# BrandonHanx/TextReID

Measured on AMD Instinct MI355X. Metric: image-text pairs/sec (train), CLIP-RN50 + BiGRU MoCo step, bs128/GPU, higher is better.
Workload: dtype f32; 1 GPU; configs[1]: CLIP-RN50 + GRU, bs128/GPU, 384x128 images, 64-token captions, MoCo queue 8192, fp32, 1xMI355X; random-init weights, synthetic inputs resident in HBM; global_batch=128, parallelism=dp1, optimizer=Adam (fused multi-tensor), step_launch=eager launches, four streams (chosen by the probe over the recorded step)

## Files before the change

include/textreid_hip.h:

```cpp
#ifndef TEXTREID_HIP_H
#define TEXTREID_HIP_H

#include <stdint.h>

#ifdef __cplusplus
extern "C" {
#endif
#if defined(__GNUC__) || defined(__clang__)
#pragma GCC visibility push(default)
#endif

#define TRID_OK 0
#define TRID_E_INVALID (-1)
#define TRID_E_UNSUPPORTED (-2)

#define TRID_VERSION 100

int trid_version(void);
const char* trid_arch(void);
const char* trid_last_error_string(void);

enum {
    TRID_A_KC = 0,
    TRID_A_MC = 1,
// ... 108 lines not shown
int trid_conv3x3_s2_eval_p16_ok(int B, int H, int W, int Cin, int Cout);
int trid_subsample2_p16(const void* x, void* out, int B, int H, int W, int C, void* stream);
int trid_global_avgpool_p16(const void* x, const float* x_amax, float* out, int B, int HW, int C, void* stream);

int trid_stem_conv1_f32(const float* img, const float* w, float* y, float* stats, int B, int Hi, int Wi, void* stream);
int trid_stem_conv1_eval_p16(const float* img, const float* w, const float* bn_scale, const float* bn_shift, void* out,
                             const float* eval_coef, const float* eval_tin, float* out_bound, float* out_tmax, int B, int Hi, int Wi,
                             int relu, void* stream);
int trid_conv3x3_wgrad_halo_rows(int H, int W, int Cin, int Cout);
int trid_conv3x3_wgrad_halo_slabs(void);
int trid_conv3x3_wgrad_halo_p16(const void* dy, const float* dy_amax, const void* x, const float* x_amax, float* dw, float* slabs,
                                int B, int H, int W, int Cin, int Cout, void* stream);
int trid_stem_conv1_wgrad_slabs(void);
int trid_stem_conv1_wgrad_f32(const float* img, const float* dy, float* dw, float* slabs, int B, int Hi, int Wi, void* stream);
int trid_conv3x3_halo_rows(int H, int W, int Cin, int Cout);
int trid_conv3x3_halo_p16(const void* x, const float* x_amax, const void* w, const float* w_amax, float* y, float* stats,
                          int B, int H, int W, int Cin, int Cout, int chunks_per_image, void* stream);
int trid_conv3x3_halo_eval_p16(const void* x, const float* x_amax, const void* w, const float* w_amax, const float* bn_scale,
                               const float* bn_shift, void* out, const float* eval_coef, const float* eval_tin, float* out_bound,
                               float* out_tmax, int B, int H, int W, int Cin, int Cout, int relu, int pool, void* stream);
int trid_conv3x3_halo_eval_pool_ok(int H, int W, int Cin, int Cout);

long long trid_bn_finalize_ws_bytes(void);
int trid_bn_finalize_f32(const float* partials, int nparts, int rows_per_part, long long M, int C,
                         const float* gamma, const float* beta, float* running_mean, float* running_var,
                         float momentum, float eps, float* mean, float* invstd, float* scale, float* shift,
                         void* ws, void* stream);
int trid_bn_eval_coeffs_f32(const float* gamma, const float* beta, const float* running_mean,
                            const float* running_var, float eps, float* scale, float* shift, int C, void* stream);
int trid_bn_eval_bound_f32(const float* partials, int nparts, int C, const float* scale, const float* shift, int relu,
                           float* bound, void* stream);
int trid_eval_bound_coefs_f32(const long long* table, int n_tensors, float* coef, void* stream);
int trid_bn_apply_f32(const float* y, const float* scale, const float* shift, const float* res,
                      const float* rscale, const float* rshift, float* out, long long M, int C, int relu,
                      uint64_t* relu_mask, float* amax, void* stream);
int trid_bn_apply_pool2_f32(const float* y, const float* scale, const float* shift, float* out, int B, int H,
                            int W, int C, int relu, float* amax, void* stream);
int trid_bn_finalize_minmax_f32(const float* partials, int nparts, int rows_per_part, long long M, int C,
                                const float* gamma, const float* beta, float* running_mean, float* running_var,
                                float momentum, float eps, float* mean, float* invstd, float* scale, float* shift,
                                int relu, float* amax_out, void* ws, void* stream);
int trid_bn_apply_p16_f32(const void* y, int y_fmt, const float* scale, const float* shift, const void* res, const float* rscale,
                          const float* rshift, int res_fmt, const float* res_amax, void* out, int fmt, long long M, int C,
                          int relu, uint64_t* relu_mask, const float* bound_a, const float* bound_b, float* bound_sum,
                          void* stream);
int trid_bn_apply_pool2_p16_f32(const void* y, const float* scale, const float* shift, int in_fmt, const float* in_amax,
                                void* out, int fmt, int B, int H, int W, int C, int relu, const float* bound, void* stream);
int trid_avgpool2_bwd_f32(const void* g, void* dx, int B, int H, int W, int C, int accumulate, int fmt, void* stream);

long long trid_bn_bwd_ws_floats(int C);
long long trid_bn_bwd_fused_ws_floats(long long M, int C);
int trid_bn_bwd_final_f32(const float* ws, const float* ws2, long long M, int C, const float* scale, float* dgamma, float* dbeta,
                          float* bound, void* stream);
int trid_bn_bwd_reduce_f32(const float* g, const float* y, const float* act, const float* mean,
                           const float* invstd, const float* scale, const float* shift, int mask_mode,
                           int pooled, int B, int H, int W, int C, float* dgamma, float* dbeta, float* ws,
                           void* stream);
int trid_bn_bwd_apply_f32(const float* g, const float* y, const float* act, const float* mean,
                          const float* invstd, const float* scale, const float* shift, const float* dgamma,
                          const float* dbeta, int mask_mode, int pooled, int B, int H, int W, int C, float* dy,
                          float* dres, float* amax, void* stream);
int trid_bn_bwd_reduce_bound_f32(const float* g, const float* y, const float* act, const float* mean,
                                 const float* invstd, const float* scale, const float* shift, int mask_mode, int pooled,
                                 int B, int H, int W, int C, float* dgamma, float* dbeta, float* ws, float* bound,
                                 void* stream);
int trid_bn_bwd_reduce_g_f32(const void* g, int g_fmt, const void* y, int y_fmt, const float* act, const float* mean,
                             const float* invstd, const float* scale, const float* shift, int mask_mode,
                             int pooled, int B, int H, int W, int C, float* dgamma, float* dbeta, float* ws,
                             void* stream);
int trid_bn_bwd_apply_p16_f32(const void* g, int g_fmt, const void* y, int y_fmt, const float* act, const float* mean, const float* invstd,
                              const float* scale, const float* shift, const float* dgamma, const float* dbeta,
                              int mask_mode, int pooled, int B, int H, int W, int C, void* dy, int fmt, void* dres,
                              const float* bound, void* stream);

int trid_bn_bwd_dual_reduce_bound_f32(const float* g, const uint64_t* relu_bits, const float* y1, const float* y2, const float* mean1,
                                      const float* invstd1, const float* scale1, const float* mean2, const float* invstd2,
                                      const float* scale2, long long M, int C, float* dgamma1, float* dgamma2, float* dbeta,
                                      float* dbeta2, float* ws, float* bound1, float* bound2, void* stream);
int trid_bn_bwd_dual_apply_p16_f32(const float* g, const uint64_t* relu_bits, const float* y1, const float* y2, const float* mean1,
                                   const float* invstd1, const float* scale1, const float* mean2, const float* invstd2,
                                   const float* scale2, const float* dgamma1, const float* dgamma2, const float* dbeta, long long M,
                                   int C, void* dy1, void* dy2, const float* bound1, const float* bound2, void* stream);

int trid_attnpool_tokens_f32(const float* x, const float* pos, float* tok, int B, int T, int C, int ldt,
                             void* stream);
int trid_attnpool_tokens_fmt_f32(const void* x, int x_fmt, const float* x_amax, const float* pos, float* tok, int B, int T,
                                 int C, int ldt, void* stream);
int trid_attnpool_tokens_bwd_f32(const float* dtok, float* dx, float* dpos, int B, int T, int C, int ldt,
                                 void* stream);
int trid_softmax_rows_f32(float* s, long long rows, int n, int ld, void* stream);
int trid_softmax_rows_bwd_f32(const float* p, const float* dp, float* ds, long long rows, int n, int ld,
                              void* stream);
int trid_colsum_f32(const float* x, float* out, long long M, int N, long long ld, int accumulate, void* stream);

int trid_embedding_gather_f32(const float* table, const int64_t* tokens, float* x, int B, int L, int ldtok, int E,
                              long long vocab, void* stream);
int trid_embedding_bwd_f32(const float* dX, const int64_t* tokens, int B, int L, int ldtok, int E, float* dtable,
                           long long vocab, long long padding_idx, void* stream);
int trid_gru_cell_fwd_f32(const float* gi, const float* gh, float* h, const int64_t* lengths, float* gates,
                          float* hprev, float* maxv, int32_t* argt, int s, int Lmax, int L, int B, int Hd,
                          long long gates_dstride, long long hprev_dstride, void* stream);
int trid_gru_max_init_f32(float* maxv, int32_t* argt, const int64_t* lengths, int Lmax, const int64_t* lmax_dev, int B,
                          int Hd, void* stream);
int trid_gru_cell_bwd_f32(const float* dout, const int32_t* argt, const float* gates, const float* hprev,
                          const int64_t* lengths, float* dh, float* dGi, float* dgh, int s, int Lmax, int L,
                          int B, int Hd, long long gates_dstride, long long hprev_dstride, long long dgh_dstride,
                          void* stream);

long long trid_gru_whh_image_bytes(int H);
int trid_gru_step_workgroups(int B, int H);
int trid_gru_pack_whh_f16(const float* w_hh, const float* w_amax, void* img_fwd, void* img_bwd, int H, void* stream);
int trid_gru_step_fwd_f32(const void* img_fwd, const float* w_amax, const void* hp_in, void* hp_out, float* h,
                          const float* gi, const int64_t* lengths, float* gates, float* hprev, float* maxv,
                          int32_t* argt, int s, int Lmax, int L, int B, int Bp, int H, long long gates_dstride,
                          long long hprev_dstride, void* stream);
int trid_gru_step_bwd_f32(const void* img_bwd, const float* w_amax, const float* dgh_in, const float* amax_in,
                          float* amax_out, const float* dout, const int32_t* argt, const float* gates,
                          const float* hprev, const int64_t* lengths, float* dh, float* dGi, float* dgh_out, int s,
                          int Lmax, int L, int B, int H, long long gates_dstride, long long hprev_dstride,
                          long long dgh_dstride, void* stream);

int trid_gru_step_seq_fwd_f32(const void* img_fwd, const float* w_amax, const void* hp_in, void* hp_out, float* h,
                              const float* gi, const int64_t* lengths, float* gates, float* hprev, float* yseq, int s,
                              int Lmax, int L, int B, int Bp, int H, long long gates_dstride, long long hprev_dstride,
                              void* stream);
int trid_gru_step_seq_bwd_f32(const void* img_bwd, const float* w_amax, const float* dgh_in, const float* amax_in,
                              float* amax_out, const float* dyseq, const float* gates, const float* hprev,
                              const int64_t* lengths, float* dh, float* dGi, float* dgh_out, int s, int Lmax, int L, int B,
                              int H, long long gates_dstride, long long hprev_dstride, long long dgh_dstride, void* stream);
int trid_gru_cell_seq_fwd_f32(const float* gi, const float* gh, float* h, const int64_t* lengths, float* gates,
                              float* hprev, float* yseq, int s, int Lmax, int L, int B, int Hd, long long gates_dstride,
                              long long hprev_dstride, void* stream);
int trid_gru_cell_seq_bwd_f32(const float* dyseq, const float* gates, const float* hprev, const int64_t* lengths,
                              float* dh, float* dGi, float* dgh, int s, int Lmax, int L, int B, int Hd,
                              long long gates_dstride, long long hprev_dstride, long long dgh_dstride, void* stream);
int trid_dropout_seq_fwd_f32(const float* y, float* x, uint8_t* keep, long long n, float p, const int64_t* state,
                             long long draw, void* stream);
int trid_dropout_seq_bwd_f32(float* dx, const uint8_t* keep, long long n, float p, void* stream);
int trid_dropout_advance(int64_t* state, long long draws, void* stream);

int trid_l2norm_rows_f32(const float* x, float* y, float* inv_norm, long long rows, int C, float eps, void* stream);
int trid_l2norm_rows_bwd_f32(const float* dy, const float* y, const float* inv_norm, float* dx, long long rows,
                             int C, int accumulate, void* stream);
int trid_queue_hit_mask(const int64_t* id_queue, const int64_t* ids, uint8_t* flag, int K, int B, void* stream);
long long trid_infonce_ws_floats(int B, int K);
int trid_infonce_rows_f32(float* S, const float* pos, const uint8_t* hit, float* loss_rows, float* dpos, int B,
                          int K, int ldS, float invT, float gscale, float* ws, void* stream);
int trid_infonce_queue_rows_f32(float* S, const float* q, const float* key, const uint8_t* hit, float* loss_rows,
                                float* dq0, int B, int K, int ldS, int C, float invT, float gscale, float* ws,
                                void* stream);
long long trid_queue_nce_ws_floats(int B, int K, int C, int nwg_hint);
int trid_queue_nce_f32(const float* v_q, const float* t_q, const float* v_key, const float* t_key,
                       const float* t_queue, const float* v_queue, const int64_t* id_queue, const int64_t* ids,
                       float* loss_rows, float* dq, int B, int K, int C, float invT, float logit_bound, float gscale,
                       int precision, int nwg_hint, float* ws, unsigned int* ticket, float* loss, float loss_scale,
                       void* stream);
int trid_amax_f32(const float* x, long long n, float* out, void* stream);
int trid_amax_multi_f32(const float* const* ptrs, const long long* sizes, int n_tensors, float* out, void* stream);
long long trid_image_pipeline_ws_bytes(int B, int max_src_h, int W);
int trid_image_pipeline_u8(const uint8_t* src, const long long* offset, const int* hw, const int* xbounds,
                           const int* xweights, const int* ybounds, const int* yweights, const int* params, int B,
                           int H, int W, int KX, int KY, int max_src_h, int pad, const float* mean3_std3_erase3_host,
                           uint8_t* ws, float* out, void* stream);
int trid_relu_bwd_f32(const float* dy, const float* act, float* dx, long long n, void* stream);
int trid_rowdot_f32(const float* x, const float* y, float* out, long long rows, int C, void* stream);
int trid_rowscale_add_f32(const float* s, const float* y, float* dx, long long rows, int C, int accumulate,
// ... 89 lines not shown
```

textreid_amd/backbones/m_resnet.py:

```python

import logging
import math
import os
from collections import OrderedDict

import torch
from torch import nn

from .. import ops


class Bottleneck(nn.Module):
    expansion = 4

    def __init__(self, inplanes, planes, stride=1):
        super().__init__()
        self.conv1 = nn.Conv2d(inplanes, planes, 1, bias=False)
        self.bn1 = nn.BatchNorm2d(planes)
        self.conv2 = nn.Conv2d(planes, planes, 3, padding=1, bias=False)
        self.bn2 = nn.BatchNorm2d(planes)
        self.avgpool = nn.AvgPool2d(stride) if stride > 1 else nn.Identity()
        self.conv3 = nn.Conv2d(planes, planes * 4, 1, bias=False)
        self.bn3 = nn.BatchNorm2d(planes * 4)
        self.relu = nn.ReLU(inplace=True)
# ... 372 lines not shown
    G[id(blk.conv3.weight)] = ws.run(lambda d_, x_: ops.conv1x1_wgrad(d_, x_, prec=P, aa=a_dyc, ba=a_ab), dyc, ab, keep=(a_dyc, a_ab)).view_as(blk.conv3.weight)
    a_dyb = ar.slot()
    dyb, dg, db, _ = ops.bn_bwd(dab, yb, stb, None, 1, pooled=stride > 1, amax=a_dyb)
    G[id(blk.bn2.weight)], G[id(blk.bn2.bias)] = dg, db
    planes = blk.conv2.out_channels
    wbt = ops.weight_transpose(_w3x3(blk.conv2), planes, 9, planes, flip=True)
    daa = ops.conv3x3(dyb, wbt, prec=P, aa=a_dyb, ba=ar.wam(blk.conv2))
    G[id(blk.conv2.weight)] = _g3x3(ws.run(lambda d_, x_: ops.conv3x3_wgrad(d_, x_, prec=P, aa=a_dyb, ba=a_aa), dyb, aa, keep=(a_dyb, a_aa)), planes, planes)
    a_dya = ar.slot()
    dya, dg, db, _ = ops.bn_bwd(daa, ya, sta, None, 1, amax=a_dya)
    G[id(blk.bn1.weight)], G[id(blk.bn1.bias)] = dg, db
    wa = blk.conv1.weight.view(blk.conv1.out_channels, -1)
    if has_down:
        wd = blk.downsample[1].weight.view(blk.downsample[1].out_channels, -1)
        dxd = ops.matmul_nn(dyd.view(-1, dyd.shape[-1]), wd, prec=P, aa=a_dyd, ba=ar.wam(blk.downsample[1])).view(xd.shape)
        G[id(blk.downsample[1].weight)] = ws.run(lambda d_, x_: ops.conv1x1_wgrad(d_, x_, prec=P, aa=a_dyd, ba=a_xd), dyd, xd, keep=(a_dyd, a_xd)).view_as(blk.downsample[1].weight)
        dx = ops.avgpool2_bwd(dxd) if stride > 1 else dxd
    else:
        dx = dres
    ops.matmul_nn(dya.view(-1, dya.shape[-1]), wa, out=dx.view(-1, dx.shape[-1]), accumulate=True, prec=P, aa=a_dya, ba=ar.wam(blk.conv1))
    G[id(blk.conv1.weight)] = ws.run(lambda d_, x_: ops.conv1x1_wgrad(d_, x_, prec=P, aa=a_dya, ba=ax), dya, x, keep=(a_dya, ax)).view_as(blk.conv1.weight)
    return dx


def block_forward_p16(blk, x, WP, dev, training, save, nbt, masks=None):
    assert training
    stride = blk.stride
    fmt = x.fmt

    def fin(bn, parts, M, relu):
        if fmt == 2:
            return _bn_coeffs(bn, parts, M, True, nbt), None
        bound = ops.amax_slot(dev)
        return _finalize_minmax(bn, parts, M, relu, bound, nbt), bound

    ya, pa = ops.conv_p16(x, WP[id(blk.conv1.weight)])
    Ma = ya.numel() // ya.shape[-1]
    sta, a_aa = fin(blk.bn1, pa, Ma, True)
    aa = ops.bn_apply_p16(ya, sta, a_aa, relu=True, fmt=fmt)
    yb, pb = ops.conv_p16(aa, WP[id(blk.conv2.weight)], conv3=True)
    stb, a_ab = fin(blk.bn2, pb, Ma, True)
    ab = ops.bn_apply_pool2_p16(yb, stb, a_ab, relu=True, fmt=fmt) if stride > 1 else ops.bn_apply_p16(yb, stb, a_ab, relu=True, fmt=fmt)
    Mc = ab.data.numel() // ab.shape[-1]
    xd = yd = std = None
    if blk.downsample is None and fmt == 1 and not save and ops.conv1x1_bn_res_ok(Mc, blk.conv3.out_channels, ab.shape[-1]):
        pc = ops.conv1x1_stats_p16(ab, WP[id(blk.conv3.weight)])
        stc, a_c = fin(blk.bn3, pc, Mc, False)
        out, rmask, yc = ops.conv1x1_bn_res_p16(ab, WP[id(blk.conv3.weight)], stc, a_c, x, relu=True, want_mask=save, keep_y=save)
        rec = (x, ya, sta, aa, yb, stb, ab, yc, stc, xd, yd, std, rmask) if save else None
        if masks is not None:
            masks.extend([aa.unpack() > 0, ab.unpack() > 0, out.unpack() > 0])
        return out, rec
    yc, pc = ops.conv_p16(ab, WP[id(blk.conv3.weight)])
    stc, a_c = fin(blk.bn3, pc, Mc, False)
    if blk.downsample is not None:
        xd = ops.bn_apply_pool2_p16(x, None, x.amax, fmt=fmt) if stride > 1 else x
        yd, pd = ops.conv_p16(xd, WP[id(blk.downsample[1].weight)])
        std, a_d = fin(blk.downsample[2], pd, Mc, False)
        out = ops.bn_apply_p16(yc, stc, a_c, relu=True, res=yd, res_st=std, bound_res=a_d, want_mask=save, fmt=fmt)
    else:
        out = ops.bn_apply_p16(yc, stc, a_c, relu=True, res=x, bound_res=x.amax, want_mask=save, fmt=fmt)
    rec = None
    if save:
        out, rmask = out
        rec = (x, ya, sta, aa, yb, stb, ab, yc, stc, xd, yd, std, rmask)
    if masks is not None:
        masks.extend([aa.unpack() > 0, (ops.bn_apply(yb.float(), stb, relu=True) if stride > 1 else ab.unpack()) > 0, out.unpack() > 0])
    return out, rec


def _finalize_minmax(bn, partials, M, relu, bound, counters, rows_per_part=ops.STATS_ROWS):
    st = ops.bn_finalize_minmax(partials, M, bn.weight, bn.bias, bn.running_mean, bn.running_var, relu, bound, rows_per_part=rows_per_part)
    counters.append(bn.num_batches_tracked)
    return st


_MASKED_ACC = _os.environ.get("TRID_MASKED_ACC", "1") != "0"


_BN3_FUSE = _os.environ.get("TRID_BN3_FUSE", "1") != "0"
_BN3_FUSE_MIN_PLANES = int(_os.environ.get("TRID_BN3_FUSE_MIN_PLANES", "256"))


def block_backward_p16(blk, rec, g, WPT, ws, G, g_sums=None, prev_rec=None, prev_blk=None):
    x, ya, sta, aa, yb, stb, ab, yc, stc, xd, yd, std, rmask = rec
    stride = blk.stride
    has_down = blk.downsample is not None

    fmt = x.fmt

    def wgrad(weight, dy, act, conv=None, post=None):
        if conv is not None and fmt == 1 and ops.conv3x3_wgrad_halo_rows(conv[0], conv[1], conv[2], dy.shape[-1]):
            fn = lambda d_, x_: ops.conv3x3_wgrad_halo_p16(ops.P16(d_, dy.amax), ops.P16(x_, act.amax))
        else:
            fn = lambda d_, x_: ops.wgrad_p16(ops.P16(d_, dy.amax, fmt), ops.P16(x_, act.amax, fmt), conv=conv)
        ws.defer(G, id(weight), fn, (dy.data, act.data), keep=(dy.amax, act.amax), post=post if post is not None else (lambda o: o.view_as(weight)))

    masked_acc = _MASKED_ACC and not has_down and g.is_contiguous()
    if has_down and ops.bn_bwd_dual_ok(g, yc, yd, fmt):
        dyc, dg, db, dyd, dg2, db2 = ops.bn_bwd_dual_p16(g, rmask, yc, stc, yd, std)
        G[id(blk.bn3.weight)], G[id(blk.bn3.bias)] = dg, db
        G[id(blk.downsample[2].weight)], G[id(blk.downsample[2].bias)] = dg2, db2
        dres = None
    else:
        dyc, dg, db, dres = ops.bn_bwd_p16(g, yc, stc, 3, act=rmask, want_dres=not has_down and not masked_acc, fmt=fmt,
                                           presummed=g_sums if (g_sums is not None and g_sums.y is yc) else None)
        G[id(blk.bn3.weight)], G[id(blk.bn3.bias)] = dg, db
        if has_down:
            dyd, dg, db, _ = ops.bn_bwd_p16(g, yd, std, 3, act=rmask, fmt=fmt)
            G[id(blk.downsample[2].weight)], G[id(blk.downsample[2].bias)] = dg, db
    planes = blk.conv2.out_channels
    Mc = dyc.data.numel() // dyc.shape[-1]
    dab = ops.empty(tuple(ab.shape), g, dtype=g.dtype)
    sums_b = ops.BnBwdSums(yb, stb) if (stride == 1 and g.dtype == torch.float32 and ops.bn_bwd_fusable(yb, Mc, planes, fmt)) else None
    ops.gemm_p16(dyc, WPT[id(blk.conv3.weight)], dab, Mc, planes, dyc.shape[-1], planes, bn_bwd=sums_b)
    wgrad(blk.conv3.weight, dyc, ab)
    dyb, dg, db, _ = ops.bn_bwd_p16(dab, yb, stb, 1, pooled=stride > 1, fmt=fmt, presummed=sums_b)
    G[id(blk.bn2.weight)], G[id(blk.bn2.bias)] = dg, db
    Bi, H, W, _ = yb.shape
    Ma = Bi * H * W
    sums_a = None
    if fmt == 1 and ops.USE_HALO_BLOCKS and ops.conv3x3_halo_rows(H, W, planes, planes):
        daa = ops.conv3x3_halo_p16(dyb, WPT[id(blk.conv2.weight)], stats=False)
    else:
        daa = ops.empty(tuple(aa.shape), g, dtype=g.dtype)
        sums_a = ops.BnBwdSums(ya, sta) if (g.dtype == torch.float32 and ops.bn_bwd_fusable(ya, Ma, planes, fmt)) else None
        ops.gemm_p16(dyb, WPT[id(blk.conv2.weight)], daa, Ma, planes, 9 * planes, planes, conv=(H, W, planes), bn_bwd=sums_a)
    wgrad(blk.conv2.weight, dyb, aa, conv=(H, W, planes), post=lambda o: _g3x3(o, planes, planes))
    dya, dg, db, _ = ops.bn_bwd_p16(daa, ya, sta, 1, fmt=fmt, presummed=sums_a)
    G[id(blk.bn1.weight)], G[id(blk.bn1.bias)] = dg, db
    cin = blk.conv1.in_channels
    if has_down:
        dxd = ops.empty(tuple(xd.shape), g, dtype=g.dtype)
        ops.gemm_p16(dyd, WPT[id(blk.downsample[1].weight)], dxd, Mc, cin, dyd.shape[-1], cin)
        wgrad(blk.downsample[1].weight, dyd, xd)
        dx = ops.avgpool2_bwd(dxd) if stride > 1 else dxd
    else:
        dx = g if masked_acc else dres
    nxt = None
    if (_BN3_FUSE and prev_rec is not None and prev_blk is not None and prev_blk.downsample is None and fmt == 1 and planes >= _BN3_FUSE_MIN_PLANES
            and dx.dtype == torch.float32 and dx.is_contiguous() and prev_rec[12] is not None
            and ops.bn_bwd_fusable(prev_rec[7], Ma, cin, fmt) and tuple(prev_rec[7].shape) == tuple(dx.shape)):
        nxt = ops.BnBwdSums(prev_rec[7], prev_rec[8], mask=prev_rec[12])
    ops.gemm_p16(dya, WPT[id(blk.conv1.weight)], dx, Ma, cin, planes, cin, accumulate=True, cmask=rmask if masked_acc else None, bn_bwd=nxt)
    wgrad(blk.conv1.weight, dya, x)
    ws.flush(block_end=True)
    return dx, nxt


class _EncoderFn(torch.autograd.Function):

    @staticmethod
    def forward(ctx, images, mod, save, *params):
        if not mod.training and not save and mod.fold_eval_bn and getattr(mod, "_debug_taps", None) is None:
            if ops.USE_EVAL_P16 and ops.USE_P16 and ops.conv_precision() == 16 and p16_eligible(mod, 32) and stem_p16_ok(mod, images):
                out, saved = mod._run_forward_eval_p16(images), None
            else:
                out, saved = mod._run_forward_folded(images), None
        else:
            if save and not mod.training:
                raise NotImplementedError("ModifiedResNet: gradients through an eval-mode (running-statistics) forward are not "
                                          "implemented; call under torch.no_grad() or in train() mode")
            out, saved = mod._run_forward(images, save)
        ctx.mod = mod
        ctx.saved = saved
        return out

    @staticmethod
    def backward(ctx, gout):
        mod, saved = ctx.mod, ctx.saved
        ctx.saved = None
        if saved is None:
            raise RuntimeError("backward through an encoder forward that did not save activations")
        grads = mod._run_backward(saved, gout.contiguous())
        return (None, None, None) + tuple(grads)


class ModifiedResNet(nn.Module):
    def __init__(self, layers, output_dim, heads, last_stride=1, input_resolution=(224, 224), width=64):
        super().__init__()
        self.output_dim = output_dim
        self.out_channels = output_dim
        self.fold_eval_bn = True
        self.grad_sync = None
        self.input_resolution = input_resolution
        self.conv1 = nn.Conv2d(3, width // 2, kernel_size=3, stride=2, padding=1, bias=False)
        self.bn1 = nn.BatchNorm2d(width // 2)
        self.conv2 = nn.Conv2d(width // 2, width // 2, kernel_size=3, padding=1, bias=False)
        self.bn2 = nn.BatchNorm2d(width // 2)
        self.conv3 = nn.Conv2d(width // 2, width, kernel_size=3, padding=1, bias=False)
        self.bn3 = nn.BatchNorm2d(width)
        self.avgpool = nn.AvgPool2d(2)
        self.relu = nn.ReLU(inplace=True)
        self._inplanes = width
        self.layer1 = self._make_layer(width, layers[0])
        self.layer2 = self._make_layer(width * 2, layers[1], stride=2)
        self.layer3 = self._make_layer(width * 4, layers[2], stride=2)
        self.layer4 = self._make_layer(width * 8, layers[3], stride=last_stride)
        embed_dim = width * 32
# ... 390 lines not shown
```

textreid_amd/ops.py:

```python

import ctypes
import os
import math

import torch

from . import lib as L
from .lib import GemmDesc, call

A_KC, A_MC, A_CONV = L.TRID_A_KC, L.TRID_A_MC, L.TRID_A_CONV
B_KC, B_NC, B_CONV = L.TRID_B_KC, L.TRID_B_NC, L.TRID_B_CONV

BN_EPS = 1e-5
BN_MOMENTUM = 0.1
STATS_ROWS = 128
GEMM_PRECISION = int(__import__("os").environ.get("TRID_GEMM_PRECISION", "6"))
CONV_PRECISION = int(__import__("os").environ.get("TRID_CONV_PRECISION", "16"))


def conv_precision():
    return CONV_PRECISION if GEMM_PRECISION == 6 else GEMM_PRECISION


_raw_stream = torch._C._cuda_getCurrentRawStream
# ... 482 lines not shown
def conv_eval_p16(x, w, st, coef, relu=True, res=None, conv3=False, pool=False):
    C = x.shape[-1]
    M = x.data.numel() // C
    N = w.shape[0]
    K = 9 * C if conv3 else C
    shape = tuple(x.shape[:-1]) + (N,)
    if pool:
        assert conv3 and res is None and conv_eval_pool_ok(x.shape[1], x.shape[2], N)
        shape = (x.shape[0], x.shape[1] // 2, x.shape[2] // 2, N)
    out = p16_empty(shape, x.data, 1)
    dev = x.data.device
    if conv3 and res is None and not pool and USE_HALO_BLOCKS and conv3x3_halo_rows(x.shape[1], x.shape[2], C, N):
        return conv3x3_halo_eval_p16(x, w, st, coef, relu)
    bound, tmax = amax_slot(dev), amax_slot(dev)
    if not conv3 and USE_STREAM and K in (64, 128, 256) and _query("trid_conv1x1_bn_res_p16_ok", int(M), int(N), int(K)):
        call("trid_conv1x1_eval_p16", _p(x.data), _p(x.amax), _p(w.data), _p(w.amax), _p(st.scale), _p(st.shift),
             _p(res.data) if res is not None else None, _p(res.amax) if res is not None else None, _p(out), _p(coef), _p(x.tmax),
             _p(res.tmax) if res is not None else None, _p(bound), _p(tmax), M, N, K, 1 if relu else 0, stream())
        return P16(out, bound, 1, tmax)
    d = GemmDesc()
    d.A, d.B, d.C = _p(x.data), _p(w.data), _p(out)
    d.M, d.N, d.K = M, N, K
    d.lda, d.ldb, d.ldc = C, K, N
    d.batch, d.splits = 1, 1
    d.a_mode, d.b_mode = (A_CONV if conv3 else A_KC), B_KC
    d.alpha = 1.0
    if conv3:
        d.H, d.W, d.Cin = x.shape[1], x.shape[2], C
    d.precision = 16
    d.a_amax, d.b_amax = _p(x.amax), _p(w.amax)
    d.relu = 1 if relu else 0
    d.c_format = 1
    d.col_scale, d.bias = _p(st.scale), _p(st.shift)
    if res is not None:
        d.res_p16, d.res_amax, d.eval_tres = _p(res.data), _p(res.amax), _p(res.tmax)
    d.eval_coef, d.eval_tin = _p(coef), _p(x.tmax)
    d.out_bound, d.out_tmax = _p(bound), _p(tmax)
    d.eval_pool_w = x.shape[2] if pool else 0
    call("trid_gemm_p16", ctypes.addressof(d), -1, stream())
    return P16(out, bound, 1, tmax)


USE_FUSED_EXPAND = __import__("os").environ.get("TRID_FUSED_EXPAND", "1") != "0"


def conv1x1_bn_res_ok(M, N, K):
    return USE_FUSED_EXPAND and USE_STREAM and K <= 128 and bool(_query("trid_conv1x1_bn_res_p16_ok", int(M), int(N), int(K)))


def conv1x1_stats_p16(x, w):
    C = x.shape[-1]
    M = x.data.numel() // C
    N = w.shape[0]
    rows = _query("trid_gemm_p16_stream_stats_rows", int(M), int(N), int(C))
    st = empty(((M + rows - 1) // rows, N, 4), x.data)
    call("trid_gemm_p16_stream", _p(x.data), _p(x.amax), _p(w.data), _p(w.amax), None, N, _p(st), M, N, C, 0, None, stream())
    return Partials(st, rows)


def conv1x1_bn_res_p16(x, w, st, bound, res, relu=True, want_mask=False, keep_y=False):
    C = x.shape[-1]
    M = x.data.numel() // C
    N = w.shape[0]
    shape = tuple(x.shape[:-1]) + (N,)
    out = p16_empty(shape, x.data, 1)
    y = empty(shape, x.data) if keep_y else None
    mask = torch.empty(((M * N // 4 + 63) // 64) * 4, dtype=torch.int64, device=x.data.device) if want_mask else None
    osum = amax_slot(x.data.device)
    call("trid_conv1x1_bn_res_p16", _p(x.data), _p(x.amax), _p(w.data), _p(w.amax), _p(y), _p(st.scale), _p(st.shift), _p(res.data), _p(res.amax),
         _p(out), _p(bound), _p(res.amax), _p(osum), _p(mask), M, N, C, 1 if relu else 0, stream())
    return P16(out, osum, 1), mask, y


def bn_apply_pool2_p16(y, st, bound, relu=True, fmt=1):
    src = y.data if isinstance(y, P16) else y
    Bi, H, W, C = src.shape
    out = p16_empty((Bi, H // 2, W // 2, C), src, fmt)
    call("trid_bn_apply_pool2_p16_f32", _p(src), _p(st.scale) if st else None, _p(st.shift) if st else None,
         y.fmt if isinstance(y, P16) else (2 if y.dtype == torch.bfloat16 else 0), _p(y.amax) if isinstance(y, P16) else None, _p(out), fmt, Bi, H, W, C,
         1 if (relu and st is not None) else 0, _p(bound), stream())
    return P16(out, bound if fmt == 1 else None, fmt, y.tmax if (isinstance(y, P16) and st is None and fmt == 1) else None)


def bn_bwd_p16(g, y, st, mask_mode, act=None, pooled=False, want_dres=False, fmt=1, presummed=None):
    Bi, H, W, C = y.shape
    dg = empty((2, C), y)
    dgamma, dbeta = dg[0], dg[1]
    bound = None
    g_fmt = 2 if g.dtype == torch.bfloat16 else 0
    y_fmt = 2 if y.dtype == torch.bfloat16 else 0
    if presummed is not None:
        assert fmt == 1 and g_fmt == 0 and y_fmt == 0 and not pooled and presummed.y is y
        assert (mask_mode == 3 and presummed.mask is act) if presummed.mask is not None else mask_mode == (1 if presummed.relu else 0)
        bound = amax_slot(y.device)
        call("trid_bn_bwd_final_f32", _p(presummed.ws), _p(presummed.ws2), presummed.M, C, _p(st.scale), _p(dgamma), _p(dbeta), _p(bound), stream())
    elif fmt == 1:
        ws = _bn_ws(C, y)
        assert g_fmt == 0 and y_fmt == 0
        bound = amax_slot(y.device)
        call("trid_bn_bwd_reduce_bound_f32", _p(g), _p(y), _p(act), _p(st.mean), _p(st.invstd), _p(st.scale), _p(st.shift),
             mask_mode, 1 if pooled else 0, Bi, H, W, C, _p(dgamma), _p(dbeta), _p(ws), _p(bound), stream())
    else:
        ws = _bn_ws(C, y)
        call("trid_bn_bwd_reduce_g_f32", _p(g), g_fmt, _p(y), y_fmt, _p(act), _p(st.mean), _p(st.invstd), _p(st.scale), _p(st.shift),
             mask_mode, 1 if pooled else 0, Bi, H, W, C, _p(dgamma), _p(dbeta), _p(ws), stream())
    dy = p16_empty(y.shape, y, fmt)
    dres = torch.empty(y.shape, dtype=g.dtype, device=y.device) if want_dres else None
    call("trid_bn_bwd_apply_p16_f32", _p(g), g_fmt, _p(y), y_fmt, _p(act), _p(st.mean), _p(st.invstd), _p(st.scale), _p(st.shift),
         _p(dgamma), _p(dbeta), mask_mode, 1 if pooled else 0, Bi, H, W, C, _p(dy), fmt, _p(dres), _p(bound), stream())
    return P16(dy, bound, fmt), dgamma, dbeta, dres


USE_BN_DUAL = os.environ.get("TRID_BN_DUAL", "1") != "0"


def bn_bwd_dual_ok(g, y1, y2, fmt=1):
    C = y1.shape[-1]
    CQ = C // 4
    return (USE_BN_DUAL and fmt == 1 and g.dtype == torch.float32 and y1.dtype == torch.float32 and y2.dtype == torch.float32 and g.is_contiguous()
            and tuple(y1.shape) == tuple(y2.shape) == tuple(g.shape) and C % 32 == 0 and (256 % CQ == 0 or CQ % 256 == 0))


def bn_bwd_dual_p16(g, bits, y1, st1, y2, st2):
    C = y1.shape[-1]
    M = y1.numel() // C
    dg = empty((4, C), y1)
    key = ("dual", C, y1.device, stream(y1.device))
    ws = _ws_cache.get(key)
    if ws is None:
        ws = empty((2 * L.load().trid_bn_bwd_ws_floats(C),), y1)
        _ws_cache[key] = ws
    b1, b2 = amax_slot(y1.device), amax_slot(y1.device)
    call("trid_bn_bwd_dual_reduce_bound_f32", _p(g), _p(bits), _p(y1), _p(y2), _p(st1.mean), _p(st1.invstd), _p(st1.scale), _p(st2.mean),
         _p(st2.invstd), _p(st2.scale), M, C, _p(dg[0]), _p(dg[1]), _p(dg[2]), _p(dg[3]), _p(ws), _p(b1), _p(b2), stream())
    dy1, dy2 = p16_empty(y1.shape, y1, 1), p16_empty(y2.shape, y2, 1)
    call("trid_bn_bwd_dual_apply_p16_f32", _p(g), _p(bits), _p(y1), _p(y2), _p(st1.mean), _p(st1.invstd), _p(st1.scale), _p(st2.mean),
         _p(st2.invstd), _p(st2.scale), _p(dg[0]), _p(dg[1]), _p(dg[2]), M, C, _p(dy1), _p(dy2), _p(b1), _p(b2), stream())
    return P16(dy1, b1, 1), dg[0], dg[2], P16(dy2, b2, 1), dg[1], dg[3]


def wgrad_p16(dy, x, conv=None, alpha=1.0):
    N = dy.shape[-1]
    M = dy.data.numel() // N
    C = x.shape[-1]
    J = 9 * C if conv is not None else C
    out = empty((N, J), dy.data)
    tiles = ((N + 127) // 128) * ((J + 127) // 128)
    splits = _wgrad_splits(tiles, M, slots=768 if N <= 64 else 512)
    d = GemmDesc()
    d.A, d.B = _p(dy.data), _p(x.data)
    d.M, d.N, d.K = N, J, M
    d.lda, d.ldb, d.ldc = N, C, J
    d.batch, d.splits = 1, splits
    d.a_mode, d.b_mode = A_MC, (B_CONV if conv is not None else B_NC)
    d.alpha = alpha
    if conv is not None:
        d.H, d.W, d.Cin = conv
    d.precision = 16 if dy.fmt == 1 else 1
    d.a_amax, d.b_amax = _p(dy.amax), _p(x.amax)
    if splits == 1:
        d.C = _p(out)
        call("trid_gemm_p16_wgrad", ctypes.addressof(d), stream())
        return out
    slab = empty((splits, N, J), dy.data)
    d.C, d.strideSplit = _p(slab), N * J
    call("trid_gemm_p16_wgrad", ctypes.addressof(d), stream())
    call("trid_slab_reduce_f32", _p(slab), _p(out), N * J, splits, N * J, 0, stream())
    return out


USE_SKINNY = os.environ.get("TRID_SKINNY_GEMM", "1") != "0"


SKINNY_MIN_K_BATCHED = 512
SKINNY_MIN_M_BATCHED = 65


def _skinny_ok(M, N, K, lda, ldb_k_contig, prec, min_k=256):
    return (USE_SKINNY and prec is None and M <= 128 and K >= min_k and K % 4 == 0 and N >= 32 and N <= 8192 and lda % 4 == 0
            and (ldb_k_contig is None or ldb_k_contig % 4 == 0))


def skinny_gemm(a, lda, b, ldb, b_mode, out, ldc, M, N, K, bias=None, alpha=1.0, accumulate=False, batch=1, strideA=0, strideB=0, strideC=0,
                strideBias=0):
    call("trid_skinny_gemm_f32", _p(a), lda, _p(b), ldb, b_mode, _p(out), ldc, _p(bias), M, N, K, alpha,
         1 if accumulate else 0, batch, strideA, strideB, strideC, strideBias, stream())


def linear(x, w, bias=None, out=None, alpha=1.0, accumulate=False, prec=None, aa=None, ba=None, relu=False):
    M, K = x.shape
    N = w.shape[0]
    if out is None:
        out = empty((M, N), x)
# ... 416 lines not shown
```

Baseline: 3128 pairs/s.

## Fuse bn3 backward apply with conv3 dgrad and wgrad into one kernel

Adds a HIP kernel for stride-1 non-downsample bottlenecks with 64 planes. It applies the bn3 backward (masked ReLU, normalisation terms) per row tile, writes dy as split fp16 into LDS, and computes both the conv3 input gradient and per-workgroup weight-gradient slabs with MFMA. A slab reduce then produces dW3. This removes the materialised dyc tensor and the separate dgrad GEMM and deferred wgrad passes over it. In exchange it drops the fused bn2 sums path (sums_b) for these blocks and keeps per-block slabs plus an extra reduction kernel.

```diff
diff --git a/include/textreid_hip.h b/include/textreid_hip.h
--- a/include/textreid_hip.h
+++ b/include/textreid_hip.h
@@ -214,6 +214,12 @@
                                    const float* scale2, const float* dgamma1, const float* dgamma2, const float* dbeta, long long M,
                                    int C, void* dy1, void* dy2, const float* bound1, const float* bound2, void* stream);
 
+int trid_bn3_bwd_conv3_p16_plan(int M, int C, int workers);
+int trid_bn3_bwd_conv3_p16(const float* g, const float* y, const uint64_t* relu_bits, const float* mean, const float* invstd,
+                           const float* scale, const float* dgamma, const float* dbeta, const float* bound, const void* ab,
+                           const float* ab_amax, const void* w, const float* w_amax, float* dab, float* slabs, int M, int C,
+                           int workers, void* stream);
+
 int trid_attnpool_tokens_f32(const float* x, const float* pos, float* tok, int B, int T, int C, int ldt,
                              void* stream);
 int trid_attnpool_tokens_fmt_f32(const void* x, int x_fmt, const float* x_amax, const float* pos, float* tok, int B, int T,
diff --git a/textreid_amd/backbones/m_resnet.py b/textreid_amd/backbones/m_resnet.py
--- a/textreid_amd/backbones/m_resnet.py
+++ b/textreid_amd/backbones/m_resnet.py
@@ -478,6 +478,10 @@
 _BN3_FUSE_MIN_PLANES = int(_os.environ.get("TRID_BN3_FUSE_MIN_PLANES", "256"))
 
 
+def bn3_conv3_fused_ok(blk, g, yc, ab, fmt):
+    return blk.downsample is None and blk.stride == 1 and ops.bn3_bwd_conv3_ok(g, yc, ab, blk.conv2.out_channels, fmt)
+
+
 def block_backward_p16(blk, rec, g, WPT, ws, G, g_sums=None, prev_rec=None, prev_blk=None):
     x, ya, sta, aa, yb, stb, ab, yc, stc, xd, yd, std, rmask = rec
     stride = blk.stride
@@ -493,7 +497,16 @@
         ws.defer(G, id(weight), fn, (dy.data, act.data), keep=(dy.amax, act.amax), post=post if post is not None else (lambda o: o.view_as(weight)))
 
     masked_acc = _MASKED_ACC and not has_down and g.is_contiguous()
-    if has_down and ops.bn_bwd_dual_ok(g, yc, yd, fmt):
+    planes = blk.conv2.out_channels
+    fused3 = bn3_conv3_fused_ok(blk, g, yc, ab, fmt) and masked_acc
+    dyc = None
+    if fused3:
+        dab, dw3, dg, db = ops.bn3_bwd_conv3_p16(g, yc, stc, rmask, ab, WPT[id(blk.conv3.weight)],
+                                                 presummed=g_sums if (g_sums is not None and g_sums.y is yc) else None)
+        G[id(blk.bn3.weight)], G[id(blk.bn3.bias)] = dg, db
+        G[id(blk.conv3.weight)] = dw3.view_as(blk.conv3.weight)
+        dres = None
+    elif has_down and ops.bn_bwd_dual_ok(g, yc, yd, fmt):
         dyc, dg, db, dyd, dg2, db2 = ops.bn_bwd_dual_p16(g, rmask, yc, stc, yd, std)
         G[id(blk.bn3.weight)], G[id(blk.bn3.bias)] = dg, db
         G[id(blk.downsample[2].weight)], G[id(blk.downsample[2].bias)] = dg2, db2
@@ -505,12 +518,14 @@
         if has_down:
             dyd, dg, db, _ = ops.bn_bwd_p16(g, yd, std, 3, act=rmask, fmt=fmt)
             G[id(blk.downsample[2].weight)], G[id(blk.downsample[2].bias)] = dg, db
-    planes = blk.conv2.out_channels
-    Mc = dyc.data.numel() // dyc.shape[-1]
-    dab = ops.empty(tuple(ab.shape), g, dtype=g.dtype)
-    sums_b = ops.BnBwdSums(yb, stb) if (stride == 1 and g.dtype == torch.float32 and ops.bn_bwd_fusable(yb, Mc, planes, fmt)) else None
-    ops.gemm_p16(dyc, WPT[id(blk.conv3.weight)], dab, Mc, planes, dyc.shape[-1], planes, bn_bwd=sums_b)
-    wgrad(blk.conv3.weight, dyc, ab)
+    Mc = yc.numel() // yc.shape[-1]
+    if fused3:
+        sums_b = None
+    else:
+        dab = ops.empty(tuple(ab.shape), g, dtype=g.dtype)
+        sums_b = ops.BnBwdSums(yb, stb) if (stride == 1 and g.dtype == torch.float32 and ops.bn_bwd_fusable(yb, Mc, planes, fmt)) else None
+        ops.gemm_p16(dyc, WPT[id(blk.conv3.weight)], dab, Mc, planes, dyc.shape[-1], planes, bn_bwd=sums_b)
+        wgrad(blk.conv3.weight, dyc, ab)
     dyb, dg, db, _ = ops.bn_bwd_p16(dab, yb, stb, 1, pooled=stride > 1, fmt=fmt, presummed=sums_b)
     G[id(blk.bn2.weight)], G[id(blk.bn2.bias)] = dg, db
     Bi, H, W, _ = yb.shape
diff --git a/textreid_amd/csrc/bn_bwd_conv_fused.hip b/textreid_amd/csrc/bn_bwd_conv_fused.hip
--- /dev/null
+++ b/textreid_amd/csrc/bn_bwd_conv_fused.hip
@@ -0,0 +1,306 @@
+
+#include <algorithm>
+#include <mutex>
+
+#include "split_common.h"
+
+namespace trid {
+
+namespace {
+
+typedef __fp16 h4v_t __attribute__((__vector_size__(4 * sizeof(__fp16))));
+
+__device__ __forceinline__ f16x8 tr_frag2(const char* lo_addr, const char* hi_addr) {
+    typedef __attribute__((address_space(3))) h4v_t* lp;
+    const h4v_t lo = __builtin_amdgcn_ds_read_tr16_b64_v4f16((lp)(lo_addr));
+    const h4v_t hi = __builtin_amdgcn_ds_read_tr16_b64_v4f16((lp)(hi_addr));
+    f16x8 r;
+    r[0] = lo[0]; r[1] = lo[1]; r[2] = lo[2]; r[3] = lo[3];
+    r[4] = hi[0]; r[5] = hi[1]; r[6] = hi[2]; r[7] = hi[3];
+    return r;
+}
+__device__ __forceinline__ void lds_sync() {
+    asm volatile("s_waitcnt lgkmcnt(0)" ::: "memory");
+    __builtin_amdgcn_s_barrier();
+    asm volatile("" ::: "memory");
+}
+__device__ __forceinline__ int dy_swz(int row) { return (((row >> 1) & 1) << 2) | ((row >> 2) & 3); }
+
+struct Bn3FuseParams {
+    const float4* g;
+    const float4* y;
+    const unsigned* bits;
+    const float4* mean;
+    const float4* invstd;
+    const float4* scale;
+    const float4* dgamma;
+    const float4* dbeta;
+    const float* bound;
+    const char* ab;
+    const float* ab_amax;
+    const char* w;
+    const float* w_amax;
+    float* dab;
+    float* slabs;
+    int M, tiles, per;
+    float invM;
+};
+
+constexpr int BN3F_RB = 64;
+
+template <int C>
+struct Bn3FuseLds {
+    static constexpr int P = C / 4, G = C / 32, GP = P / 32;
+    static constexpr int GB = BN3F_RB * 128 + 64;
+    static constexpr int GBAB = BN3F_RB * 128;
+    static constexpr int RP = P + 4;
+    static constexpr int DY = 0, AB = G * GB, RED = AB + GP * GBAB;
+    static constexpr int BYTES = RED + 4 * BN3F_RB * RP * 4;
+};
+
+template <int C, bool NT>
+__global__ __launch_bounds__(512) void bn3_bwd_conv3_kernel(Bn3FuseParams p) {
+    static_assert(C == 256, "one row of C / 4 channel quads per wave instruction; W3^T and dW3 in 32 + 32 registers per lane");
+    typedef Bn3FuseLds<C> L;
+    constexpr int P = L::P, RB = BN3F_RB, RPW = RB / 8;
+    extern __shared__ __attribute__((aligned(16))) uint4 smem[];
+    char* const sDY = reinterpret_cast<char*>(smem) + L::DY;
+    char* const sAB = reinterpret_cast<char*>(smem) + L::AB;
+    float* const sRED = reinterpret_cast<float*>(reinterpret_cast<char*>(smem) + L::RED);
+
+    const int tid = threadIdx.x, lane = tid & 63;
+    const int wave = __builtin_amdgcn_readfirstlane(tid >> 6);
+    const int kh = lane >> 5;
+    const int pn = wave & 1, kc = wave >> 1;
+
+    const int t_begin = blockIdx.x * p.per, t_end = min(p.tiles, t_begin + p.per);
+
+    const float oscale = f16_scale_of(*p.bound);
+    const float un_d = 1.f / (oscale * f16_scale_of(*p.w_amax));
+    const float un_w = 1.f / (oscale * f16_scale_of(*p.ab_amax));
+
+    f16x8 bw[2][2][2];
+    {
+        const char* br = p.w + (size_t)(32 * pn + (lane & 31)) * (C * 4);
+#pragma unroll
+        for (int gg = 0; gg < 2; ++gg)
+#pragma unroll
+            for (int ks = 0; ks < 2; ++ks)
+#pragma unroll
+                for (int pl = 0; pl < 2; ++pl)
+                    bw[gg][ks][pl] = __builtin_bit_cast(f16x8, *reinterpret_cast<const uint4*>(br + (2 * kc + gg) * 128 + (4 * pl + 2 * ks + kh) * 16));
+    }
+    const float4 mu = p.mean[lane], is = p.invstd[lane], sc = p.scale[lane], dg = p.dgamma[lane], db = p.dbeta[lane];
+    const float invM = p.invM;
+
+    v16f accw[2];
+#pragma unroll
+    for (int n = 0; n < 2; ++n)
+#pragma unroll
+        for (int r = 0; r < 16; ++r) accw[n][r] = 0.f;
+
+    typedef unsigned v4u __attribute__((ext_vector_type(4)));
+    v4u gq[RPW], yq[RPW], abq[2];
+    unsigned mk = 0;
+    const __amdgpu_buffer_rsrc_t rsG = __builtin_amdgcn_make_buffer_rsrc((void*)p.g, 0, (unsigned)((size_t)p.M * C * 4), 0x00020000);
+    const __amdgpu_buffer_rsrc_t rsY = __builtin_amdgcn_make_buffer_rsrc((void*)p.y, 0, (unsigned)((size_t)p.M * C * 4), 0x00020000);
+    const __amdgpu_buffer_rsrc_t rsM = __builtin_amdgcn_make_buffer_rsrc((void*)p.bits, 0, (unsigned)((size_t)p.M * (C / 8)), 0x00020000);
+    const __amdgpu_buffer_rsrc_t rsA = __builtin_amdgcn_make_buffer_rsrc((void*)p.ab, 0, (unsigned)((size_t)p.M * P * 4), 0x00020000);
+    auto fetch = [&](int t) {
+        const unsigned r0 = (unsigned)(t * RB + RPW * wave);
+        mk = __builtin_amdgcn_raw_buffer_load_b32(rsM, (unsigned)lane * 4u, r0 * (unsigned)(C / 8), 0);
+#pragma unroll
+        for (int j = 0; j < RPW; ++j) {
+            const unsigned so = (r0 + (unsigned)j) * (unsigned)(C * 4);
+            gq[j] = __builtin_amdgcn_raw_buffer_load_b128(rsG, (unsigned)lane * 16u, so, NT ? 2 : 0);
+            yq[j] = __builtin_amdgcn_raw_buffer_load_b128(rsY, (unsigned)lane * 16u, so, NT ? 2 : 0);
+        }
+#pragma unroll
+        for (int j = 0; j < 2; ++j)
+            abq[j] = __builtin_amdgcn_raw_buffer_load_b128(rsA, (unsigned)tid * 16u, (unsigned)(t * RB) * (unsigned)(P * 4) + 8192u * (unsigned)j, 0);
+    };
+
+    const int h2 = (lane >> 4) & 1, r4 = (lane & 15) >> 2, c8 = lane & 3;
+    const int fr = dy_swz(lane & 31);
+
+    if (t_begin < t_end) fetch(t_begin);
+    for (int t = t_begin; t < t_end; ++t) {
+        {
+            const int g8 = lane >> 3, qi = lane & 7;
+#pragma unroll
+            for (int j = 0; j < RPW; ++j) {
+                const int rl = RPW * wave + j;
+                const bool valid = t * RB + rl < p.M;
+                const int sh = lane & 31;
+                const unsigned w0 = (unsigned)__shfl((int)mk, j * 8 + 0 + kh, 64), w1 = (unsigned)__shfl((int)mk, j * 8 + 2 + kh, 64);
+                const unsigned w2 = (unsigned)__shfl((int)mk, j * 8 + 4 + kh, 64), w3 = (unsigned)__shfl((int)mk, j * 8 + 6 + kh, 64);
+                float4 gm = make_float4(__uint_as_float(gq[j][0]), __uint_as_float(gq[j][1]), __uint_as_float(gq[j][2]), __uint_as_float(gq[j][3]));
+                const float4 yv = make_float4(__uint_as_float(yq[j][0]), __uint_as_float(yq[j][1]), __uint_as_float(yq[j][2]), __uint_as_float(yq[j][3]));
+                gm.x = ((w0 >> sh) & 1u) ? gm.x : 0.f; gm.y = ((w1 >> sh) & 1u) ? gm.y : 0.f;
+                gm.z = ((w2 >> sh) & 1u) ? gm.z : 0.f; gm.w = ((w3 >> sh) & 1u) ? gm.w : 0.f;
+                const float4 xh = make_float4((yv.x - mu.x) * is.x, (yv.y - mu.y) * is.y, (yv.z - mu.z) * is.z, (yv.w - mu.w) * is.w);
+                float4 o;
+                o.x = sc.x * (gm.x - db.x * invM - xh.x * dg.x * invM);
+                o.y = sc.y * (gm.y - db.y * invM - xh.y * dg.y * invM);
+                o.z = sc.z * (gm.z - db.z * invM - xh.z * dg.z * invM);
+                o.w = sc.w * (gm.w - db.w * invM - xh.w * dg.w * invM);
+                if (!valid) o = make_float4(0.f, 0.f, 0.f, 0.f);
+                unsigned h0, l0, h1, l1;
+                f16_split2(o.x * oscale, o.y * oscale, h0, l0);
+                f16_split2(o.z * oscale, o.w * oscale, h1, l1);
+                const int f = dy_swz(rl);
+                char* dst = sDY + g8 * L::GB + rl * 128 + 8 * (qi & 1);
+                *reinterpret_cast<uint2*>(dst + (((qi >> 1) ^ f) << 4)) = make_uint2(h0, h1);
+                *reinterpret_cast<uint2*>(dst + (((4 + (qi >> 1)) ^ f) << 4)) = make_uint2(l0, l1);
+            }
+#pragma unroll
+            for (int j = 0; j < 2; ++j) {
+                const int u = tid + 512 * j;
+                const int rl = u / (P / 4), s = u % (P / 4);
+                const int swz = ((rl >> 1) & 1) << 2;
+                *reinterpret_cast<v4u*>(sAB + (s >> 3) * L::GBAB + rl * 128 + (((s & 7) ^ swz) << 4)) = abq[j];
+            }
+        }
+        lds_sync();
+        if (t + 1 < t_end) fetch(t + 1);
+        __builtin_amdgcn_sched_barrier(0);
+
+        v16f accd[2];
+#pragma unroll
+        for (int i = 0; i < 2; ++i)
+#pragma unroll
+            for (int r = 0; r < 16; ++r) accd[i][r] = 0.f;
+#pragma unroll
+        for (int gg = 0; gg < 2; ++gg)
+#pragma unroll
+            for (int ks = 0; ks < 2; ++ks) {
+                f16x8 a[2][2];
+#pragma unroll
+                for (int i = 0; i < 2; ++i) {
+                    const char* base = sDY + (2 * kc + gg) * L::GB + (32 * i + (lane & 31)) * 128;
+                    a[i][0] = __builtin_bit_cast(f16x8, *reinterpret_cast<const uint4*>(base + (((2 * ks + kh) ^ fr) << 4)));
+                    a[i][1] = __builtin_bit_cast(f16x8, *reinterpret_cast<const uint4*>(base + (((4 + 2 * ks + kh) ^ fr) << 4)));
+                }
+#pragma unroll
+                for (int i = 0; i < 2; ++i) accd[i] = __builtin_amdgcn_mfma_f32_32x32x16_f16(a[i][0], bw[gg][ks][1], accd[i], 0, 0, 0);
+#pragma unroll
+                for (int i = 0; i < 2; ++i) accd[i] = __builtin_amdgcn_mfma_f32_32x32x16_f16(a[i][1], bw[gg][ks][0], accd[i], 0, 0, 0);
+#pragma unroll
+                for (int i = 0; i < 2; ++i) accd[i] = __builtin_amdgcn_mfma_f32_32x32x16_f16(a[i][0], bw[gg][ks][0], accd[i], 0, 0, 0);
+            }
+#pragma unroll
+        for (int ks = 0; ks < 4; ++ks) {
+            const int pix0 = 16 * ks + 8 * kh + r4, pix1 = pix0 + 4;
+            f16x8 a[2], b[2][2];
+#pragma unroll
+            for (int pl = 0; pl < 2; ++pl) {
+                const int slot = pl * 4 + h2 * 2 + (c8 >> 1);
+                const char* gbase = sDY + wave * L::GB + 8 * (c8 & 1);
+                a[pl] = tr_frag2(gbase + pix0 * 128 + ((slot ^ dy_swz(pix0)) << 4), gbase + pix1 * 128 + ((slot ^ dy_swz(pix1)) << 4));
+                const int sab = (slot ^ ((r4 >> 1) << 2)) << 4;
+#pragma unroll
+                for (int n = 0; n < 2; ++n) {
+                    const char* bb = sAB + n * L::GBAB + pix0 * 128 + sab + 8 * (c8 & 1);
+                    b[pl][n] = tr_frag2(bb, bb + 512);
+                }
+            }
+#pragma unroll
+            for (int n = 0; n < 2; ++n) accw[n] = __builtin_amdgcn_mfma_f32_32x32x16_f16(a[0], b[1][n], accw[n], 0, 0, 0);
+#pragma unroll
+            for (int n = 0; n < 2; ++n) accw[n] = __builtin_amdgcn_mfma_f32_32x32x16_f16(a[1], b[0][n], accw[n], 0, 0, 0);
+#pragma unroll
+            for (int n = 0; n < 2; ++n) accw[n] = __builtin_amdgcn_mfma_f32_32x32x16_f16(a[0], b[0][n], accw[n], 0, 0, 0);
+        }
+        {
+            float* dst = sRED + (kc * RB + 4 * kh) * L::RP + 32 * pn + (lane & 31);
+#pragma unroll
+            for (int i = 0; i < 2; ++i)
+#pragma unroll
+                for (int r = 0; r < 16; ++r) dst[(32 * i + (r & 3) + 8 * (r >> 2)) * L::RP] = accd[i][r];
+        }
+        lds_sync();
+        {
+            constexpr int TPR = P / 8;
+            const int rl = tid / TPR, p0 = 8 * (tid % TPR);
+            float4 s0 = make_float4(0.f, 0.f, 0.f, 0.f), s1 = s0;
+#pragma unroll
+            for (int q = 0; q < 4; ++q) {
+                const float4* src = reinterpret_cast<const float4*>(sRED + (q * RB + rl) * L::RP + p0);
+                const float4 u = src[0], v = src[1];
+                s0.x += u.x; s0.y += u.y; s0.z += u.z; s0.w += u.w;
+                s1.x += v.x; s1.y += v.y; s1.z += v.z; s1.w += v.w;
+            }
+            const long long row = (long long)t * RB + rl;
+            if (row < p.M) {
+                float4* out = reinterpret_cast<float4*>(p.dab + row * P + p0);
+                out[0] = make_float4(s0.x * un_d, s0.y * un_d, s0.z * un_d, s0.w * un_d);
+                out[1] = make_float4(s1.x * un_d, s1.y * un_d, s1.z * un_d, s1.w * un_d);
+            }
+        }
+    }
+
+    {
+        float* slab = p.slabs + (size_t)blockIdx.x * (C * P) + (size_t)(32 * wave + 4 * kh) * P + (lane & 31);
+#pragma unroll
+        for (int n = 0; n < 2; ++n)
+#pragma unroll
+            for (int r = 0; r < 16; ++r) slab[((r & 3) + 8 * (r >> 2)) * P + 32 * n] = accw[n][r] * un_w;
+    }
+}
+
+}
+
+}
+
+using namespace trid;
+
+extern "C" int trid_bn3_bwd_conv3_p16_plan(int M, int C, int workers) {
+    if (C != 256 || M <= 0 || (long long)M * C * 4 >= (1ll << 31)) return 0;
+    const int tiles = (M + BN3F_RB - 1) / BN3F_RB;
+    int w = workers > 0 ? workers : 256;
+    if (w > tiles) w = tiles;
+    const int per = (tiles + w - 1) / w;
+    return (tiles + per - 1) / per;
+}
+
+extern "C" int trid_bn3_bwd_conv3_p16(const float* g, const float* y, const uint64_t* relu_bits, const float* mean, const float* invstd,
+                                      const float* scale, const float* dgamma, const float* dbeta, const float* bound, const void* ab,
+                                      const float* ab_amax, const void* w, const float* w_amax, float* dab, float* slabs, int M, int C,
+                                      int workers, void* stream) {
+    TRID_REQUIRE(g && y && relu_bits && mean && invstd && scale && dgamma && dbeta && bound && ab && ab_amax && w && w_amax && dab && slabs,
+                 "trid_bn3_bwd_conv3_p16: null pointer");
+    const int wgs = trid_bn3_bwd_conv3_p16_plan(M, C, workers);
+    const bool nt = (long long)M * C * 4 >= STREAM_NT_MIN_BYTES;
+    TRID_REQUIRE(wgs > 0, "trid_bn3_bwd_conv3_p16: C = 256 (planes 64) only (M=%d C=%d)", M, C);
+    TRID_REQUIRE(aligned16(g) && aligned16(y) && aligned16(relu_bits) && aligned16(ab) && aligned16(w) && aligned16(dab) && aligned16(slabs) &&
+                     aligned16(mean) && aligned16(invstd) && aligned16(scale) && aligned16(dgamma) && aligned16(dbeta),
+                 "trid_bn3_bwd_conv3_p16: operands must be 16-byte aligned");
+    Bn3FuseParams p;
+    memset(&p, 0, sizeof(p));
+    p.g = reinterpret_cast<const float4*>(g); p.y = reinterpret_cast<const float4*>(y);
+    p.bits = reinterpret_cast<const unsigned*>(relu_bits);
+    p.mean = reinterpret_cast<const float4*>(mean); p.invstd = reinterpret_cast<const float4*>(invstd);
+    p.scale = reinterpret_cast<const float4*>(scale);
+    p.dgamma = reinterpret_cast<const float4*>(dgamma); p.dbeta = reinterpret_cast<const float4*>(dbeta);
+    p.bound = bound;
+    p.ab = (const char*)ab; p.ab_amax = ab_amax; p.w = (const char*)w; p.w_amax = w_amax;
+    p.dab = dab; p.slabs = slabs;
+    p.M = M;
+    p.tiles = (M + BN3F_RB - 1) / BN3F_RB;
+    p.per = (p.tiles + wgs - 1) / wgs;
+    p.invM = 1.f / (float)M;
+    constexpr int lds = Bn3FuseLds<256>::BYTES;
+    static std::once_flag once;
+    static hipError_t attr_err = hipSuccess;
+    std::call_once(once, [] {
+        attr_err = hipFuncSetAttribute((const void*)bn3_bwd_conv3_kernel<256, false>, hipFuncAttributeMaxDynamicSharedMemorySize, lds);
+        if (attr_err == hipSuccess) attr_err = hipFuncSetAttribute((const void*)bn3_bwd_conv3_kernel<256, true>, hipFuncAttributeMaxDynamicSharedMemorySize, lds);
+    });
+    if (attr_err != hipSuccess) {
+        set_error("trid_bn3_bwd_conv3_p16: cannot reserve %d B of LDS: %s", lds, hipGetErrorString(attr_err));
+        return (int)attr_err;
+    }
+    if (nt) hipLaunchKernelGGL((bn3_bwd_conv3_kernel<256, true>), dim3(wgs), dim3(512), lds, (hipStream_t)stream, p);
+    else hipLaunchKernelGGL((bn3_bwd_conv3_kernel<256, false>), dim3(wgs), dim3(512), lds, (hipStream_t)stream, p);
+    return check_launch("trid_bn3_bwd_conv3_p16");
+}
diff --git a/textreid_amd/ops.py b/textreid_amd/ops.py
--- a/textreid_amd/ops.py
+++ b/textreid_amd/ops.py
@@ -588,25 +588,34 @@
     return P16(out, bound if fmt == 1 else None, fmt, y.tmax if (isinstance(y, P16) and st is None and fmt == 1) else None)
 
 
-def bn_bwd_p16(g, y, st, mask_mode, act=None, pooled=False, want_dres=False, fmt=1, presummed=None):
+def _bn_bwd_sums_p16(g, y, st, mask_mode, act, pooled, presummed):
     Bi, H, W, C = y.shape
     dg = empty((2, C), y)
     dgamma, dbeta = dg[0], dg[1]
+    bound = amax_slot(y.device)
+    if presummed is not None:
+        assert g.dtype == torch.float32 and y.dtype == torch.float32 and not pooled and presummed.y is y
+        assert (mask_mode == 3 and presummed.mask is act) if presummed.mask is not None else mask_mode == (1 if presummed.relu else 0)
+        call("trid_bn_bwd_final_f32", _p(presummed.ws), _p(presummed.ws2), presummed.M, C, _p(st.scale), _p(dgamma), _p(dbeta), _p(bound), stream())
+    else:
+        ws = _bn_ws(C, y)
+        assert g.dtype == torch.float32 and y.dtype == torch.float32
+        call("trid_bn_bwd_reduce_bound_f32", _p(g), _p(y), _p(act), _p(st.mean), _p(st.invstd), _p(st.scale), _p(st.shift),
+             mask_mode, 1 if pooled else 0, Bi, H, W, C, _p(dgamma), _p(dbeta), _p(ws), _p(bound), stream())
+    return dgamma, dbeta, bound
+
+
+def bn_bwd_p16(g, y, st, mask_mode, act=None, pooled=False, want_dres=False, fmt=1, presummed=None):
+    Bi, H, W, C = y.shape
     bound = None
     g_fmt = 2 if g.dtype == torch.bfloat16 else 0
     y_fmt = 2 if y.dtype == torch.bfloat16 else 0
-    if presummed is not None:
-        assert fmt == 1 and g_fmt == 0 and y_fmt == 0 and not pooled and presummed.y is y
-        assert (mask_mode == 3 and presummed.mask is act) if presummed.mask is not None else mask_mode == (1 if presummed.relu else 0)
-        bound = amax_slot(y.device)
-        call("trid_bn_bwd_final_f32", _p(presummed.ws), _p(presummed.ws2), presummed.M, C, _p(st.scale), _p(dgamma), _p(dbeta), _p(bound), stream())
-    elif fmt == 1:
-        ws = _bn_ws(C, y)
-        assert g_fmt == 0 and y_fmt == 0
-        bound = amax_slot(y.device)
-        call("trid_bn_bwd_reduce_bound_f32", _p(g), _p(y), _p(act), _p(st.mean), _p(st.invstd), _p(st.scale), _p(st.shift),
-             mask_mode, 1 if pooled else 0, Bi, H, W, C, _p(dgamma), _p(dbeta), _p(ws), _p(bound), stream())
+    if fmt == 1:
+        dgamma, dbeta, bound = _bn_bwd_sums_p16(g, y, st, mask_mode, act, pooled, presummed)
     else:
+        assert presummed is None
+        dg = empty((2, C), y)
+        dgamma, dbeta = dg[0], dg[1]
         ws = _bn_ws(C, y)
         call("trid_bn_bwd_reduce_g_f32", _p(g), g_fmt, _p(y), y_fmt, _p(act), _p(st.mean), _p(st.invstd), _p(st.scale), _p(st.shift),
              mask_mode, 1 if pooled else 0, Bi, H, W, C, _p(dgamma), _p(dbeta), _p(ws), stream())
@@ -615,6 +624,44 @@
     call("trid_bn_bwd_apply_p16_f32", _p(g), g_fmt, _p(y), y_fmt, _p(act), _p(st.mean), _p(st.invstd), _p(st.scale), _p(st.shift),
          _p(dgamma), _p(dbeta), mask_mode, 1 if pooled else 0, Bi, H, W, C, _p(dy), fmt, _p(dres), _p(bound), stream())
     return P16(dy, bound, fmt), dgamma, dbeta, dres
+
+
+USE_BN3_CONV3_FUSE = os.environ.get("TRID_BN3_CONV3_FUSE", "1") != "0"
+
+
+def bn3_bwd_conv3_plan(M, C, workers=0):
+    return _query("trid_bn3_bwd_conv3_p16_plan", int(M), int(C), int(workers))
+
+
+def bn3_bwd_conv3_ok(g, yc, ab, planes, fmt):
+    if not (USE_BN3_CONV3_FUSE and fmt == 1 and planes == 64 and isinstance(ab, P16) and ab.fmt == 1):
+        return False
+    C = yc.shape[-1]
+    M = yc.numel() // C
+    return (g.dtype == torch.float32 and yc.dtype == torch.float32 and g.is_contiguous() and yc.is_contiguous() and C == 4 * planes
+            and tuple(g.shape) == tuple(yc.shape) and ab.shape[-1] == planes and ab.data.numel() == M * planes
+            and bn3_bwd_conv3_plan(M, C) > 0)
+
+
+def bn3_bwd_conv3_p16(g, yc, st, rmask, ab, w, workers=0, presummed=None):
+    C = yc.shape[-1]
+    M = yc.numel() // C
+    planes = C // 4
+    dgamma, dbeta, bound = _bn_bwd_sums_p16(g, yc, st, 3, rmask, False, presummed)
+    n = bn3_bwd_conv3_plan(M, C, workers)
+    if n <= 0:
+        raise RuntimeError("bn3_bwd_conv3_p16: shape not covered (M=%d C=%d)" % (M, C))
+    key = ("bn3conv3", M, C, int(workers), yc.device, stream(yc.device))
+    slabs = _ws_cache.get(key)
+    if slabs is None:
+        slabs = empty((n, C, planes), yc)
+        _ws_cache[key] = slabs
+    dab = empty(tuple(ab.shape), yc)
+    dw = empty((C, planes), yc)
+    call("trid_bn3_bwd_conv3_p16", _p(g), _p(yc), _p(rmask), _p(st.mean), _p(st.invstd), _p(st.scale), _p(dgamma), _p(dbeta), _p(bound),
+         _p(ab.data), _p(ab.amax), _p(w.data), _p(w.amax), _p(dab), _p(slabs), M, C, int(workers), stream())
+    call("trid_slab_reduce_f32", _p(slabs), _p(dw), C * planes, n, C * planes, 0, stream())
+    return dab, dw, dgamma, dbeta
 
 
 USE_BN_DUAL = os.environ.get("TRID_BN_DUAL", "1") != "0"
```

Result: no change. 3158 pairs/s (median of 6 runs) (+1.0%).
